# aurianer/DLA-Future

Measured on AMD Instinct MI355X. Metric: fp64 Cholesky TFlop/s, higher is better.
Workload: dtype f64

## Files before the change

### dla_future_amd/csrc/device/device_api.hpp

```cpp
#pragma once
#include <hip/hip_runtime.h>

#include "common.hpp"

namespace dlaf_mi355x {

inline hipError_t zero_device_now(void* p, size_t bytes) {
  hipError_t e = hipMemsetAsync(p, 0, bytes, nullptr);
  if (e == hipSuccess)
    e = hipStreamSynchronize(nullptr);
  return e;
}


constexpr int kDiagBlock = 64;
constexpr int kInfoSchedulingFailure = -1000000;

template <class T>
struct UpdateArgs {
  T* c;
  long c_tsr, c_tsc;
  int ldc;
  const T* a;
  long a_ts;
  int lda;
  const T* b;
  long b_ts;
  int ldb;
  int il0, il1, jl0, jl1;
  int nb, K;
  int pr, ri, pc, ci;
  int nt, last_rows;
  const int* info;
  int rect = 0;
  int nt_c = 0, last_cols = 0;
  int b_period = 1;
  long b_ts2 = 0;
  int b_jl0 = -1;
  int K1 = 0;
  const T* a2 = nullptr;
  const T* b2 = nullptr;
  int her2k = 0;
};
template <class T>
void launch_update(const UpdateArgs<T>& args, hipStream_t stream, int role = 0, long max_blocks = 0,
                   unsigned* counters = nullptr, bool counters_are_zero = false, long excl_slots = 0);
template <class T>
int update_blocks_per_cu();

template <class T>
struct TrsmArgs {
  T* b;
  long b_ts;
  int ldb;
  int il0, il1;
  int pr, ri;
  int nb, nt, last_rows;
  const T* l;
  int ldl;
  const T* winv;
  int n;
  const int* info;
  int upper = 0;
  int prio = 0;
};
template <class T>
void launch_trsm(const TrsmArgs<T>& args, hipStream_t stream);

template <class T>
void launch_potrf_diag(T* a, int lda, int jb, T* winv_block, int* info, int info_base, hipStream_t stream,
                       bool factor = true, bool upper = false, bool unit = false);

template <class T>
void launch_invert_diag_blocks(const T* tile, int ld, int kb, T* winv, int* info, hipStream_t stream, bool upper,
                               bool unit);

template <class T>
void launch_potrf_coop(T* tile, int ld, int kb, T* winv, int* info, int info_base, unsigned* sync,
                       hipStream_t stream, bool sync_is_zero = false, bool count_strips = true);
void update_launch_stats(long* persistent, long* exclusive);
unsigned long long* potrf_coop_trace_buffer();
inline size_t potrf_coop_sync_words(int kb) {
  const size_t g = (size_t) ((kb + kDiagBlock - 1) / kDiagBlock);
  return g + g * g;
}

template <class T>
struct LayoutArgs {
  T* tiles;
  T* cm;
  long ld_cm;
  int ltr, ltc;
  int nb;
  long rows, cols;
  int pr, ri, pc, ci;
  int transpose;
  int full = 0, conj = 0, scale = 0;
  T alpha{};
  int jl_first = 0, jl_count = 0;
  int rev_rows = 0, rev_cols = 0;
};
template <class T>
void launch_to_tiles(const LayoutArgs<T>& args, hipStream_t stream);
template <class T>
void launch_from_tiles(const LayoutArgs<T>& args, hipStream_t stream);

template <class T>
void launch_copy2d(T* dst, long ldd, const T* src, long lds, int rows, int cols, int transpose, int mask,
                   hipStream_t stream);

template <class T>
void launch_tile_xform(T* dst, long ldd, long dstride, const T* src, long lds, long sstride, int rows, int cols,
// ... 16 lines not shown
```

### dla_future_amd/csrc/device/kernels_potrf_coop.hip

```cpp
#include <cstdio>
#include <cstdlib>

#include "potrf_diag_core.hpp"

namespace dlaf_mi355x {

constexpr int kCB = kDiagBlock;

template <class T>
struct CoopCfg {
  using R = real_t<T>;
  static constexpr bool CX = TypeInfo<T>::is_complex;
  static constexpr int NPL = CX ? 2 : 1;
  static constexpr bool REGA = CX && sizeof(R) == 8;
  static constexpr int PAD = 16;
  static constexpr int LD = kCB + PAD;
  static constexpr int IMG = kCB * LD;
  static constexpr int OPERANDS = (REGA ? 1 : 2) * NPL * IMG;
  static constexpr int DIAG = diag_lds_elems<T, REGA>();
  static constexpr int ELEMS = OPERANDS > DIAG ? OPERANDS : DIAG;
  static constexpr int LDS_BYTES = ELEMS * (int) sizeof(R);
  static_assert(!REGA || LDS_BYTES <= 95 * 1024, "must fit beside one bulk-update workgroup");
};

// ... 538 lines not shown
        }
      }
      coop_poison_winv<T>(winv + (long) s * kCB * kCB);
      coop_publish(&flag[s], kCoopFailed, false);
      return;
    }
    T* Ws = winv + (long) s * kCB * kCB;
    for (int idx = t; idx < kPD * kPD; idx += kThreads) {
      const int rr = idx % kPD, cl = idx / kPD;
      if (rr < jb && cl < jb && rr >= cl) {
        R imv = 0;
        if constexpr (C::CX)
          imv = Lim[cl * kPDLd + rr];
        Ass[rr + (long) cl * ld] = make_el<T>(Lre[cl * kPDLd + rr], imv);
      }
      R wre = 0, wim = 0;
      if (rr < jb && cl < jb) {
        wre = diag_w_get<PACK>(Wre, PACK ? diag_wd_re<T, PACK>(Wre) : nullptr, rr, cl);
        if constexpr (C::CX)
          wim = diag_w_get<PACK>(Wim, PACK ? diag_wd_im<T, PACK>(Wre) : nullptr, rr, cl);
      }
      store_wt(&Ws[rr + (long) cl * kPD], make_el<T>(wre, wim));
    }
    coop_publish(&flag[s], 1u, false);
    if (trace != nullptr && s < 2 && t == 0)
      trace[16 + s * 8 + 6] = 4;
  }
}

template <class T>
__global__ __launch_bounds__(kThreads, 2) void potrf_coop_kernel(T* __restrict__ tile, int ld, int kb,
                                                                  T* __restrict__ winv, int* info, int info_base,
                                                                  unsigned* sync, long spin_limit, int prio, int* cu_busy,
                                                                  unsigned long long* trace) {
  int* mine = nullptr;
  if (cu_busy != nullptr && threadIdx.x == 0) {
    unsigned xcc;
    const unsigned key = phys_cu_key(xcc);
    mine = cu_busy + (xcc * 256u + key);
    atomicAdd(mine, 1);
  }
  potrf_coop_body<T>(tile, ld, kb, winv, info, info_base, sync, spin_limit, prio, trace);
  __syncthreads();
  if (mine != nullptr)
    atomicSub(mine, 1);
}

static int coop_wave_prio() {
  static const int p = [] {
    const char* e = std::getenv("DLAF_MI355X_POTRF_PRIO");
    return e ? std::atoi(e) : 1;
  }();
  return p;
}

int* cu_busy_table();

static unsigned long long* g_potrf_trace = nullptr;
unsigned long long* potrf_coop_trace_buffer() {
  static const bool on = [] {
    const char* e = std::getenv("DLAF_MI355X_POTRF_TRACE");
    return e && std::atoi(e) != 0;
  }();
  if (on && g_potrf_trace == nullptr) {
    if (hipMalloc(reinterpret_cast<void**>(&g_potrf_trace), 32 * sizeof(unsigned long long)) != hipSuccess ||
        zero_device_now(g_potrf_trace, 32 * sizeof(unsigned long long)) != hipSuccess) {
      (void) hipGetLastError();
      g_potrf_trace = nullptr;
    }
  }
  return g_potrf_trace;
}

static void fatal_device_config(const char* what) {
  std::fprintf(stderr, "[dlaf_mi355x] %s\n", what);
  std::abort();
}

template <class T>
void launch_potrf_coop(T* tile, int ld, int kb, T* winv, int* info, int info_base, unsigned* sync,
                       hipStream_t stream, bool sync_is_zero, bool count_strips) {
  if (kb <= 0)
    return;
  const int G = (kb + kCB - 1) / kCB;
  if (G > kThreads)
    fatal_device_config("potrf_coop: more than 256 strips per tile");
  if (!sync_is_zero)
    (void) hipMemsetAsync(sync, 0, sizeof(unsigned) * ((size_t) G + (size_t) G * G), stream);
  hipLaunchKernelGGL((potrf_coop_kernel<T>), dim3((unsigned) G), dim3(kThreads), CoopCfg<T>::LDS_BYTES, stream, tile, ld,
                     kb, winv, info, info_base, sync, coop_spin_limit(), coop_wave_prio(), count_strips ? cu_busy_table() : nullptr,
                     info_base == 0 ? potrf_coop_trace_buffer() : nullptr);
}

template <class T>
static void coop_init_one() {
  (void) hipFuncSetAttribute(reinterpret_cast<const void*>(&potrf_coop_kernel<T>),
                             hipFuncAttributeMaxDynamicSharedMemorySize, CoopCfg<T>::LDS_BYTES);
}

void potrf_coop_kernels_init() {
  coop_init_one<float>();
  coop_init_one<double>();
  coop_init_one<cfloat>();
  coop_init_one<cdouble>();
}

template void launch_potrf_coop<float>(float*, int, int, float*, int*, int, unsigned*, hipStream_t, bool, bool);
template void launch_potrf_coop<double>(double*, int, int, double*, int*, int, unsigned*, hipStream_t, bool, bool);
template void launch_potrf_coop<cfloat>(cfloat*, int, int, cfloat*, int*, int, unsigned*, hipStream_t, bool, bool);
template void launch_potrf_coop<cdouble>(cdouble*, int, int, cdouble*, int*, int, unsigned*, hipStream_t, bool, bool);

}
```

### dla_future_amd/csrc/device/kernels_update.hip

```cpp
#include <algorithm>
#include <cstdio>
#include <cstdlib>
#include <cstring>
#include <type_traits>
#include <utility>
#include <vector>

#include "device_api.hpp"
#include "mma_core.hpp"

namespace dlaf_mi355x {

template <class T>
struct UpdateCfg;
template <>
struct UpdateCfg<float> {
  using type = BlockCfg<float, 128, 128, 64, 64, 16>;
  static constexpr int min_waves = 2;
};
template <>
struct UpdateCfg<double> {
#if defined(DLAF_UPD_BIG)
  using type = BlockCfg<double, 256, 128, 64, 64, 16, true, DLAF_UPD_BIG, 512>;
  static constexpr int min_waves = 2;
// ... 10 lines not shown
};
template <>
struct UpdateCfg<cfloat> {
  using type = BlockCfg<cfloat, 128, 128, 64, 64, 16>;
  static constexpr int min_waves = 2;
};
template <>
struct UpdateCfg<cdouble> {
  using type = BlockCfg<cdouble, 128, 64, 64, 32, 8, true, 3>;
  static constexpr int min_waves = 2;
};

constexpr int kMaxPatchCols = 256;

struct UpdateMap {
  int ps;
  int psc;
  int PR;
  int tri;
  int PC;
  int colstart[kMaxPatchCols + 1];
  int xcd;
  int RB, CB;
  int bpt_m, bpt_n;
  long total;
  int persist;
  unsigned* counters;
  int lockstep;
  unsigned kphase_ticks;
  int excl_rank;
  unsigned excl_budget;
  int steal;
  int* cu_busy;
};

__device__ unsigned char g_cu_rank[8][256];

__global__ void cu_probe_kernel(unsigned* seen) {
  extern __shared__ unsigned char probe_lds[];
  if (threadIdx.x == 0) {
    unsigned xcc;
    const unsigned key = phys_cu_key(xcc);
    atomicOr(&seen[xcc * 8 + (key >> 5)], 1u << (key & 31));
    probe_lds[0] = (unsigned char) key;
  }
  for (int i = 0; i < 64; ++i)
    __builtin_amdgcn_s_sleep(64);
}

template <class T, bool VEC, bool UTAIL = false, int PART = 0>
__device__ __forceinline__ void update_block(const UpdateArgs<T>& p, const UpdateMap& mp, long w,
                                             real_t<T>* __restrict__ lds, int s0 = 0) {
  using Cfg = typename UpdateCfg<T>::type;
  using R = real_t<T>;

  const int ps = mp.ps, psc = mp.psc;
  const long patch = w >> (ps + psc);
  const int q = (int) (w & ((1 << (ps + psc)) - 1));
  int pi, pj;
  if (mp.tri) {
    int lo = 0, hi = mp.PC;
    while (hi - lo > 1) {
      const int mid = (lo + hi) >> 1;
      if (mp.colstart[mid] <= patch)
        lo = mid;
      else
        hi = mid;
// ... 249 lines not shown
            const T cv = col[ml];
            if constexpr (Cfg::CX) {
              T r{cv.re - acc.re[i][j][v], cv.im - acc.im[i][j][v]};
              if (diag && (m0 + ml) == (n0 + nl))
                r.im = R(0);
              col[ml] = r;
            }
            else {
              col[ml] = cv - acc.re[i][j][v];
            }
          }
        }
      }
    }
  }
}

template <class T, bool VEC, int ROLE>
__global__ __launch_bounds__(UpdateCfg<T>::type::THREADS, UpdateCfg<T>::min_waves) void update_kernel(UpdateArgs<T> p,
                                                                                                     UpdateMap mp) {
  using R = real_t<T>;
  extern __shared__ __attribute__((aligned(16))) unsigned char lds_raw[];
  R* lds = reinterpret_cast<R*>(lds_raw);
  if (*p.info != 0)
    return;
  if (!mp.persist) {
    const long v = blockIdx.x;
    const long w = mp.xcd ? (v & 7) * (mp.total >> 3) + (v >> 3) : v;
#ifdef DLAF_UPD_LEAN
    update_block<T, VEC, false, (ROLE == 0 ? 1 : 0)>(p, mp, w, lds);
#else
    update_block<T, VEC>(p, mp, w, lds);
#endif
    return;
  }
  __shared__ unsigned next_item;
  const int nq = mp.xcd ? 8 : 1;
  const long per_q = mp.total / nq;
  const int q0 = mp.xcd ? (int) (blockIdx.x & 7) : 0;
  const unsigned W = gridDim.x / nq;
  if (mp.excl_rank > 0) {
    __shared__ int leave;
    if (threadIdx.x == 0) {
      unsigned xcc;
      const unsigned key = phys_cu_key(xcc);
      leave = 0;
      if ((int) g_cu_rank[xcc][key] < mp.excl_rank)
        leave = atomicAdd(&mp.counters[15], 1u) < mp.excl_budget ? 1 : 0;
    }
    __syncthreads();
    if (leave)
      return;
  }
  __shared__ int next_s0;
  const int nslab = p.K / UpdateCfg<T>::type::BK;
  int q = q0, tried = 1;
  int* my_busy = nullptr;
  if (mp.cu_busy != nullptr && threadIdx.x == 0) {
    unsigned xcc;
    const unsigned key = phys_cu_key(xcc);
    my_busy = mp.cu_busy + (xcc * 256u + key);
  }
  for (;;) {
    if (threadIdx.x == 0) {
      if (my_busy != nullptr) {
        int spins = 0;
        while (__hip_atomic_load(my_busy, __ATOMIC_RELAXED, __HIP_MEMORY_SCOPE_AGENT) > 0 && ++spins < 4000)
          __builtin_amdgcn_s_sleep(64);
      }
      next_item = atomicAdd(&mp.counters[q], 1u);
      next_s0 = (mp.kphase_ticks != 0 && nslab > 1) ? (int) ((wall_clock64() / mp.kphase_ticks) % (unsigned) nslab) : 0;
    }
    __syncthreads();
#if DLAF_GLDS_SCALAR_ADDR
    const long i = (long) (unsigned) __builtin_amdgcn_readfirstlane((int) next_item);
    const int s0 = __builtin_amdgcn_readfirstlane(next_s0);
#else
    const long i = next_item;
    const int s0 = next_s0;
#endif
    __syncthreads();
    if (i >= per_q) {
      if (!mp.steal || tried >= nq)
        break;
      ++tried;
      q = (q + 1) % nq;
      continue;
    }
    if (mp.lockstep) {
      if (threadIdx.x == 0) {
        const unsigned need = (unsigned) (i / W) * W;
        long spins = 0;
        while (__hip_atomic_load(&mp.counters[8 + q], __ATOMIC_RELAXED, __HIP_MEMORY_SCOPE_AGENT) < need && ++spins < 2000000)
          __builtin_amdgcn_s_sleep(8);
      }
      __syncthreads();
    }
#ifdef DLAF_UPD_LEAN
    update_block<T, VEC, ROLE == 0, (ROLE == 0 ? 1 : 0)>(p, mp, (long) q * per_q + i, lds, s0);
#else
    update_block<T, VEC, ROLE == 0>(p, mp, (long) q * per_q + i, lds, s0);
#endif
    if (mp.lockstep && threadIdx.x == 0)
      __hip_atomic_fetch_add(&mp.counters[8 + q], 1u, __ATOMIC_RELAXED, __HIP_MEMORY_SCOPE_AGENT);
  }
}

static bool update_lockstep() {
  static const bool on = [] {
    const char* e = std::getenv("DLAF_MI355X_LOCKSTEP");
    return e ? std::atoi(e) != 0 : false;
  }();
  return on;
}

template <class T>
static unsigned kphase_ticks(int resident) {
  using Cfg = typename UpdateCfg<T>::type;
  static const double rate = [] {
    const char* on = std::getenv("DLAF_MI355X_KPHASE");
    if (on == nullptr || std::atoi(on) == 0)
      return 0.0;
    if (const char* e = std::getenv("DLAF_MI355X_KPHASE_RATE"))
      return std::atof(e) * 1e12;
    return (sizeof(real_t<T>) == 8 ? 66.5e12 : 120e12);
  }();
  static const double khz = [] {
    int dev = 0, v = 0;
    (void) hipGetDevice(&dev);
    if (hipDeviceGetAttribute(&v, hipDeviceAttributeWallClockRate, dev) != hipSuccess || v <= 0)
      v = 100000;
    return (double) v;
  }();
  if (rate <= 0 || resident <= 0)
    return 0;
// ... 11 lines not shown
static int* g_cu_busy = nullptr;
int* cu_busy_table() {
  static const bool on = [] {
    const char* e = std::getenv("DLAF_MI355X_POTRF_YIELD");
    return e ? std::atoi(e) != 0 : true;
  }();
  if (on && g_cu_busy == nullptr) {
    if (hipMalloc(reinterpret_cast<void**>(&g_cu_busy), 8 * 256 * sizeof(int)) != hipSuccess ||
        zero_device_now(g_cu_busy, 8 * 256 * sizeof(int)) != hipSuccess) {
      (void) hipGetLastError();
      g_cu_busy = nullptr;
    }
  }
  return g_cu_busy;
}

static int g_probe_xcds = 0, g_probe_cus_per_xcd = 0, g_probe_engines = 1;

static long g_launch_stats[2] = {0, 0};
void update_launch_stats(long* persistent, long* exclusive) {
  *persistent = g_launch_stats[0];
  *exclusive = g_launch_stats[1];
}

static bool update_steal() {
  static const bool on = [] {
    const char* e = std::getenv("DLAF_MI355X_STEAL");
    return e ? std::atoi(e) != 0 : true;
  }();
  return on;
}

template <class T>
void launch_update(const UpdateArgs<T>& a, hipStream_t stream, int role, long max_blocks, unsigned* counters,
                   bool counters_are_zero, long excl_slots) {
  using Cfg = typename UpdateCfg<T>::type;
  if (a.il1 <= a.il0 || a.jl1 <= a.jl0 || a.K <= 0 || a.nb <= 0)
    return;
  UpdateMap mp;
  mp.bpt_m = (a.nb + Cfg::BM - 1) / Cfg::BM;
  mp.bpt_n = (a.nb + Cfg::BN - 1) / Cfg::BN;
  mp.RB = (a.il1 - a.il0) * mp.bpt_m;
  mp.CB = (a.jl1 - a.jl0) * mp.bpt_n;
  static_assert(Cfg::BM % Cfg::BN == 0 && ((Cfg::BM / Cfg::BN) & (Cfg::BM / Cfg::BN - 1)) == 0, "BM = 2^s * BN");
  constexpr int kAspectShift = (Cfg::BM / Cfg::BN == 1) ? 0 : (Cfg::BM / Cfg::BN == 2) ? 1 : 2;
  const bool big = (mp.RB >= 16 && mp.CB >= 16);
  mp.ps = big ? 3 : 0;
  mp.psc = big ? 3 + kAspectShift : 0;
  mp.PR = (mp.RB + (1 << mp.ps) - 1) >> mp.ps;
  mp.PC = (mp.CB + (1 << mp.psc) - 1) >> mp.psc;
  long npatch = (long) mp.PR * mp.PC;
  mp.tri = 0;
  if (mp.PC <= kMaxPatchCols) {
    mp.tri = 1;
    mp.colstart[0] = 0;
    for (int pj = 0; pj < mp.PC; ++pj) {
      const int jl_min = a.jl0 + (pj << mp.psc) / mp.bpt_n;
      const long gj_min = (long) jl_min * a.pc + a.ci;
      long il_first = (gj_min - a.ri + a.pr - 1) / a.pr;
      if (gj_min <= a.ri || a.rect)
        il_first = 0;
      if (il_first < a.il0)
        il_first = a.il0;
      int cnt = 0;
      if (il_first < a.il1) {
        const int pi0 = (int) (((il_first - a.il0) * mp.bpt_m) >> mp.ps);
        cnt = mp.PR - pi0;
      }
      mp.colstart[pj + 1] = mp.colstart[pj] + cnt;
    }
    npatch = mp.colstart[mp.PC];
    if (npatch == 0)
      return;
  }
  mp.total = npatch << (mp.ps + mp.psc);
  mp.xcd = (mp.ps > 0) ? 1 : 0;
  long grid = mp.total;
  mp.persist = 0;
  mp.lockstep = 0;
  mp.kphase_ticks = 0;
  mp.counters = nullptr;
  mp.excl_rank = 0;
  mp.excl_budget = 0;
  mp.steal = 0;
  long excl_rank = 0;
  if (excl_slots > 0) {
    static const int per_cu = update_blocks_per_cu<T>();
    const long round = (long) per_cu * g_probe_xcds * g_probe_engines;
    if (g_probe_xcds > 0 && !update_lockstep() && excl_slots % round == 0 &&
        (excl_slots / round) * g_probe_engines <= g_probe_cus_per_xcd / 2)
      excl_rank = (excl_slots / round) * g_probe_engines;
    else {
      max_blocks = std::max<long>(8, max_blocks - excl_slots);
      excl_slots = 0;
    }
  }
  if (max_blocks > 0 && counters != nullptr && mp.total > max_blocks) {
    grid = mp.xcd ? (max_blocks / 8) * 8 : max_blocks;
    if (grid < 8)
      grid = 8;
    mp.persist = 1;
    mp.counters = counters;
    mp.lockstep = update_lockstep() ? 1 : 0;
    mp.kphase_ticks = kphase_ticks<T>((int) (grid));
    mp.steal = (update_steal() && !mp.lockstep) ? 1 : 0;
    mp.cu_busy = (role == 0) ? g_cu_busy : nullptr;
    ++g_launch_stats[0];
    if (excl_rank > 0) {
      mp.excl_rank = (int) excl_rank;
      mp.excl_budget = (unsigned) excl_slots;
      ++g_launch_stats[1];
    }
    if (!counters_are_zero)
      (void) hipMemsetAsync(counters, 0, 16 * sizeof(unsigned), stream);
  }
  const bool vec = aligned16<T>(a.a, a.lda) && aligned16<T>(a.a, a.a_ts) && aligned16<T>(a.b, a.ldb) &&
                   aligned16<T>(a.b, a.b_ts) && aligned16<T>(a.b, a.b_ts2) &&
                   (a.K1 == 0 || (aligned16<T>(a.a2, 0) && aligned16<T>(a.b2, 0)));
  auto go = [&](auto vtag, auto rtag) {
    constexpr bool V = decltype(vtag)::value;
    constexpr int RL = decltype(rtag)::value;
    hipLaunchKernelGGL((update_kernel<T, V, RL>), dim3((unsigned) grid), dim3(Cfg::THREADS), Cfg::LDS_BYTES, stream, a, mp);
  };
  auto by_role = [&](auto vtag) {
    switch (role) {
      case 0: go(vtag, std::integral_constant<int, 0>{}); break;
      case 1: go(vtag, std::integral_constant<int, 1>{}); break;
      case 3: go(vtag, std::integral_constant<int, 3>{}); break;
      default: go(vtag, std::integral_constant<int, 2>{}); break;
    }
  };
  if (vec)
    by_role(std::true_type{});
  else
    by_role(std::false_type{});
}

template <class T>
int update_blocks_per_cu() {
  using Cfg = typename UpdateCfg<T>::type;
  int n = 0;
  if (hipOccupancyMaxActiveBlocksPerMultiprocessor(&n, reinterpret_cast<const void*>(&update_kernel<T, true, 0>), Cfg::THREADS,
                                                   Cfg::LDS_BYTES) != hipSuccess || n < 1)
    n = 1;
  return n;
}

template <class T>
static void update_init_one() {
  using Cfg = typename UpdateCfg<T>::type;
#define SET_ONE(V, RL)                                                                         \
  (void) hipFuncSetAttribute(reinterpret_cast<const void*>(&update_kernel<T, V, RL>),           \
                             hipFuncAttributeMaxDynamicSharedMemorySize, Cfg::LDS_BYTES)
  SET_ONE(true, 0);
  SET_ONE(true, 1);
  SET_ONE(true, 2);
  SET_ONE(true, 3);
  SET_ONE(false, 0);
  SET_ONE(false, 1);
  SET_ONE(false, 2);
  SET_ONE(false, 3);
#undef SET_ONE
}

static void probe_compute_units() {
  const bool verbose = [] {
    const char* e = std::getenv("DLAF_MI355X_PROBE_VERBOSE");
    return e && std::atoi(e) != 0;
// ... 56 lines not shown
    max_engines = std::max(max_engines, engines);
    {
      std::vector<unsigned> sorted(keys.size());
      for (size_t r = 0; r < idx.size(); ++r)
        sorted[r] = keys[idx[r]];
      keys.swap(sorted);
    }
    if (verbose) {
      std::fprintf(stderr, "[dlaf_mi355x] compute-unit probe: XCD %d: %zu compute units:", x, keys.size());
      for (unsigned k : keys)
        std::fprintf(stderr, " %u.%u.%u", k >> 5, (k >> 4) & 1u, k & 15u);
      std::fprintf(stderr, "\n");
    }
  }
  if (xcds == 0)
    return note("no compute unit seen", hipSuccess);
  err = hipMemcpyToSymbol(HIP_SYMBOL(g_cu_rank), rank, sizeof(rank));
  if (err != hipSuccess)
    return note("hipMemcpyToSymbol", err);
  g_probe_xcds = xcds;
  g_probe_cus_per_xcd = min_cus;
  g_probe_engines = std::max(1, max_engines);
}

void update_kernels_init() {
  update_init_one<float>();
  update_init_one<double>();
  update_init_one<cfloat>();
  update_init_one<cdouble>();
  probe_compute_units();
  (void) cu_busy_table();
}

template void launch_update<float>(const UpdateArgs<float>&, hipStream_t, int, long, unsigned*, bool, long);
template int update_blocks_per_cu<float>();
template void launch_update<double>(const UpdateArgs<double>&, hipStream_t, int, long, unsigned*, bool, long);
template int update_blocks_per_cu<double>();
template void launch_update<cfloat>(const UpdateArgs<cfloat>&, hipStream_t, int, long, unsigned*, bool, long);
template int update_blocks_per_cu<cfloat>();
template void launch_update<cdouble>(const UpdateArgs<cdouble>&, hipStream_t, int, long, unsigned*, bool, long);
template int update_blocks_per_cu<cdouble>();

}
```

### dla_future_amd/csrc/host/cholesky.cpp

```cpp
#include "runtime.hpp"

#include <algorithm>
#include <cstdlib>
#include <cstring>
#include <vector>

namespace dlaf_mi355x {

static bool potrf_use_chain() {
  static const bool chain = [] {
    const char* e = std::getenv("DLAF_MI355X_POTRF");
    return e && std::strcmp(e, "chain") == 0;
  }();
  return chain;
}

template <class T>
void potrf_tile(T* t, int ld, int kb, T* winv, int* info, int info_base, unsigned* sync, hipStream_t s) {
  constexpr int JB = kDiagBlock;
  if (!potrf_use_chain()) {
    launch_potrf_coop(t, ld, kb, winv, info, info_base, sync, s,  true,  true);
    return;
  }
  for (int j0 = 0; j0 < kb; j0 += JB) {
    const int jb = std::min(JB, kb - j0);
    T* djj = t + j0 + (size_t) j0 * ld;
    T* wj = winv + (size_t) (j0 / JB) * JB * JB;
    launch_potrf_diag(djj, ld, jb, wj, info, info_base + j0, s);
    const int rem = kb - j0 - jb;
    if (rem <= 0)
      break;
    T* sub = t + (j0 + jb) + (size_t) j0 * ld;
    TrsmArgs<T> ta;
    ta.b = sub;
    ta.b_ts = 0;
    ta.ldb = ld;
    ta.il0 = 0;
    ta.il1 = 1;
    ta.pr = 1;
    ta.ri = 0;
    ta.nb = rem;
    ta.nt = 1;
    ta.last_rows = rem;
    ta.l = djj;
    ta.ldl = ld;
    ta.winv = wj;
    ta.n = jb;
    ta.info = info;
    launch_trsm(ta, s);
    UpdateArgs<T> ua;
    ua.c = t + (j0 + jb) + (size_t) (j0 + jb) * ld;
    ua.c_tsr = ua.c_tsc = 0;
    ua.ldc = ld;
    ua.a = sub;
    ua.a_ts = 0;
    ua.lda = ld;
// ... 153 lines not shown
  }

  StepT one_panel(long k, long il_n, long jl_n, const T* a_base) const {
    return StepT::one_panel(m.rows.tile_extent(k), il_n, jl_n, a_base, m.tile_elems);
  }

  void update_work(long il0, long il1, long j0, long j1, int kb, double& flops, double& bytes) const {
    flops = bytes = 0;
    const double cx = TypeInfo<T>::is_complex ? 4.0 : 1.0;
    for (long jl = j0; jl < j1; ++jl) {
      const long gj = m.cols.global_of(jl);
      const double nj = m.rows.tile_extent(gj);
      for (long il = std::max(il0, m.rows.next_local(gj)); il < il1; ++il) {
        const long gi = m.rows.global_of(il);
        const double mi = m.rows.tile_extent(gi);
        if (gi == gj) {
          flops += cx * mi * (mi + 1) * kb;
          bytes += (mi * kb + mi * mi) * sizeof(T);
        }
        else {
          flops += cx * 2.0 * mi * nj * kb;
          bytes += (mi * kb + nj * kb + 2.0 * mi * nj) * sizeof(T);
        }
      }
    }
  }

  double column_flops(const StepT& st, long jl) const {
    double f, by;
    update_work(std::max(st.il_n, m.rows.next_local(m.cols.global_of(jl))), m.ltr, jl, jl + 1, st.kb, f, by);
    return f;
  }

  void update(const StepT& st, long j0, long j1, hipStream_t s, int role, long reserve, long il_from = -1,
              long il_to = -1, int kind = -1) {
    if (!st.valid || j0 >= j1)
      return;
    const long il0 = std::max(std::max(st.il_n, il_from), m.rows.next_local(m.cols.global_of(j0)));
    const long il1 = il_to < 0 ? m.ltr : std::min(il_to, m.ltr);
    if (il0 >= il1)
      return;
    UpdateArgs<T> ua;
    ua.c = m.tiles;
    ua.c_tsr = (long) m.tile_elems;
    ua.c_tsc = (long) (m.tile_elems * m.ltr);
    ua.ldc = m.nb;
    ua.a = st.a_base + (size_t) (il0 - st.il_n) * m.tile_elems;
    ua.a_ts = (long) m.tile_elems;
    ua.lda = m.nb;
    ua.b = st.b_base;
    ua.b_ts = st.b_ts;
    ua.b_period = st.b_period;
    ua.b_ts2 = st.b_ts2;
    ua.b_jl0 = (int) st.jl_n;
    if (st.k1 > 0) {
      ua.K1 = st.k1;
      ua.a2 = st.a2_base + (size_t) (il0 - st.il_n) * m.tile_elems;
      ua.b2 = st.b2_base;
    }
    ua.ldb = m.nb;
    ua.il0 = (int) il0;
    ua.il1 = (int) il1;
    ua.jl0 = (int) j0;
    ua.jl1 = (int) j1;
    ua.nb = m.nb;
    ua.K = st.kb;
    ua.pr = m.rows.P;
    ua.ri = m.rows.shift();
    ua.pc = m.cols.P;
    ua.ci = m.cols.shift();
    ua.nt = (int) m.nt;
    ua.last_rows = last_rows;
    ua.info = m.info;
    double fl, by;
    update_work(il0, il1, j0, j1, st.kb, fl, by);
    const int pk = kind < 0 ? role : kind;
    m.prof_begin(pk, s);
    unsigned* cnt = m.coop_sync;
    bool zero = false;
    if (reserve > 0) {
      const size_t sl = std::min(next_update_slice, m.coop_sync_update_slices - 1);
      cnt = m.coop_sync + 16 * sl;
      zero = next_update_slice < m.coop_sync_update_slices - 1;
      ++next_update_slice;
    }
    static const bool exclusive = [] {
      const char* e = std::getenv("DLAF_MI355X_EXCLUSIVE_CUS");
      return e ? std::atoi(e) != 0 : true;
    }();
    if (reserve > 0 && exclusive)
      launch_update(ua, s, role, m.bulk_slots, cnt, zero, reserve);
    else
      launch_update(ua, s, role, reserve > 0 ? std::max<long>(8, m.bulk_slots - reserve) : 0, cnt, zero);
    DLAF_HIP_CHECK(hipGetLastError());
    m.prof_end(pk, s, fl, by);
  }

  void trsm(long il0, long il1, long klc, const T* Lkk, const T* Wkk, int kb, hipStream_t ts = nullptr) {
    if (ts == nullptr)
      ts = s_main;
    if (il0 >= il1)
      return;
    TrsmArgs<T> ta;
    ta.b = m.tile(il0, klc);
    ta.b_ts = (long) m.tile_elems;
    ta.ldb = m.nb;
    ta.il0 = (int) il0;
    ta.il1 = (int) il1;
    ta.pr = m.rows.P;
    ta.ri = m.rows.shift();
    ta.nb = m.nb;
    ta.nt = (int) m.nt;
    ta.last_rows = last_rows;
    ta.l = Lkk;
    ta.ldl = m.nb;
    ta.winv = Wkk;
    ta.n = kb;
    ta.info = m.info;
    ta.prio = (ts != s_main) ? 1 : 0;
    double fl = 0, by = 0;
    for (long il = il0; il < il1; ++il) {
      const double mi = m.rows.tile_extent(m.rows.global_of(il));
      fl += (TypeInfo<T>::is_complex ? 4.0 : 1.0) * (double) kb * kb * mi;
      by += (0.5 * kb * kb + 2.0 * mi * kb) * sizeof(T);
    }
    m.prof_begin(2, ts);
    launch_trsm(ta, ts);
    DLAF_HIP_CHECK(hipGetLastError());
    m.prof_end(2, ts, fl, by);
  }

  T* winv_of(long k) const { return m.winv + (size_t) (k & 1) * m.winv_elems(); }
  T* diag_ws_of(long k) const { return m.diag_ws + (size_t) (k & 1) * (m.tile_elems + m.winv_elems()); }
  void potrf(long k) {
    if (m.rows.rank != m.rows.owner(k) || m.cols.rank != m.cols.owner(k))
      return;
    const int kb = m.rows.tile_extent(k);
    const double cxf = TypeInfo<T>::is_complex ? 4.0 : 1.0;
    m.prof_begin(3, s_panel);
    potrf_tile(m.tile(m.rows.local_of(k), m.cols.local_of(k)), m.nb, kb, winv_of(k), m.info, (int) (k * m.nb),
               m.coop_sync + 16 * m.coop_sync_update_slices + m.coop_sync_potrf_words * (size_t) k, s_panel);
    DLAF_HIP_CHECK(hipGetLastError());
    m.prof_end(3, s_panel, cxf * (double) kb * kb * kb / 3.0, (double) kb * kb * sizeof(T));
  }

  void diag_bcast(long k, bool in_row, bool in_col, const T*& Lkk, const T*& Wkk) {
    Lkk = Wkk = nullptr;
    if (in_row && in_col) {
      Lkk = m.tile(m.rows.local_of(k), m.cols.local_of(k));
      Wkk = winv_of(k);
    }
    if (in_col && m.rows.P > 1) {
      T* ws = diag_ws_of(k);
      if (in_row) {
        DLAF_HIP_CHECK(hipMemcpyAsync(ws, Lkk, tile_bytes, hipMemcpyDeviceToDevice, s_panel));
        DLAF_HIP_CHECK(hipMemcpyAsync(ws + m.tile_elems, Wkk, m.winv_elems() * sizeof(T), hipMemcpyDeviceToDevice, s_panel));
      }
      DLAF_HIP_CHECK(hipEventRecord(m.ev_diag[k], s_panel));
      DLAF_HIP_CHECK(hipStreamWaitEvent(s_comm, m.ev_diag[k], 0));
      tr->bcast(ax_col, m.rows.owner(k), m.rows.rank, ws, ws, tile_bytes + m.winv_elems() * sizeof(T), s_comm);
      DLAF_HIP_CHECK(hipEventRecord(m.ev_diag[k], s_comm));
      Lkk = ws;
      Wkk = ws + m.tile_elems;
    }
    else {
      DLAF_HIP_CHECK(hipEventRecord(m.ev_diag[k], s_panel));
    }
  }

  void transposed_panel(StepT& cur, int buf) {
    if (m.rows.P > 1) {
      m.bcast_transposed_panel(tr, ax_col, cur.a_base, cur.il_n, cur.jl_n, m.panelT[buf], s_comm, cur.b_period,
                               cur.b_ts2);
      cur.b_base = m.panelT[buf];
// ... 36 lines not shown
        continue;
      const double t = t_of(cand);
      if (t < best_t) {
        best_t = t;
        best = cand;
      }
    }
    return best;
  }

  bool u1_on_main(long k, long slots, double bulk_flops) const {
    using R = PairRates<T>;
    const long nb = m.nb;
    const double cxf = TypeInfo<T>::is_complex ? 4.0 : 1.0;
    const double below1 = (double) std::max<long>(0, m.n - (k + 1) * nb), below2 = (double) std::max<long>(0, m.n - (k + 2) * nb);
    const double fl_chain = cxf * (double) nb * nb * (below1 + below2) + cxf * 2.0 * (double) nb * nb * below1;
    const double nblk = (double) nb / kDiagBlock;
    const double t_chain = 2.0 * nblk * nblk * R::t_potrf_blk2 + fl_chain / (R::r_trsm_slot * (double) slots);
    const double t_bulk = bulk_flops / (R::r_bulk * (1.0 - (double) slots / (double) m.bulk_slots));
    return t_bulk < t_chain;
  }

  void issue_pairs();
  void issue_sidecar();
  void issue_early();
  void issue_classic();
};

template <class T>
void CholeskyIssue<T>::issue_pairs() {
  constexpr double kSplitFrac = 0.3;
  const long nt = m.nt, ltr = m.ltr, ltc = m.ltc;
  StepT prev;
  for (long k = 0; k < nt; k += 2) {
    if (tr)
      tr->mark(k);
    if (k >= 2)
      DLAF_HIP_CHECK(hipStreamWaitEvent(s_panel, m.ev_high[k - 2], 0));
    potrf(k);
    const bool second = k + 1 < nt;
    const bool more = k + 2 < nt;
    if (second) {
      trsm(k + 1, ltr, k, m.tile(k, k), winv_of(k), m.rows.tile_extent(k), s_panel);
      panel_done(k, s_panel);
    }
    const bool bulk = prev.valid && prev.rest0 < ltc;
    std::vector<double> colfl;
    double bulk_flops = 0;
    for (long jl = bulk ? prev.rest0 : ltc; jl < ltc; ++jl) {
      colfl.push_back(column_flops(prev, jl));
      bulk_flops += colfl.back();
    }
    const long slots = bulk ? pair_slots(k, bulk_flops) : kSidecarSlots;
    const bool u1_main = second && (!bulk || u1_on_main(k, slots, bulk_flops));
    long splitA = prev.rest0;
    if (u1_main && bulk) {
      double acc = 0;
      while (splitA < ltc && acc < kSplitFrac * bulk_flops)
        acc += colfl[(size_t) (splitA++ - prev.rest0)];
    }
    update(prev, prev.rest0, splitA, s_main, 0, slots);
    if (second) {
      const StepT u1 = one_panel(k, k + 1, k + 1, m.tile(k + 1 < ltr ? k + 1 : 0, k));
      if (u1_main) {
        DLAF_HIP_CHECK(hipStreamWaitEvent(s_main, m.ev_panel[k], 0));
        update(u1, k + 1, k + 2, s_main, 1, 0);
        DLAF_HIP_CHECK(hipEventRecord(m.ev_head[k], s_main));
        DLAF_HIP_CHECK(hipStreamWaitEvent(s_panel, m.ev_head[k], 0));
      }
      else {
        update(u1, k + 1, k + 2, s_panel, 1, 0);
      }
      potrf(k + 1);
      if (more) {
        trsm(k + 2, ltr, k + 1, m.tile(k + 1, k + 1), winv_of(k + 1), m.rows.tile_extent(k + 1), s_panel);
        panel_done(k + 1, s_panel);
      }
    }
    update(prev, splitA, ltc, s_main, 0, slots);
    if (!more) {
      join_last_diag(k);
      break;
    }
    DLAF_HIP_CHECK(hipStreamWaitEvent(s_main, m.ev_panel[k + 1], 0));
    StepT cur = StepT::two_panels(m.rows.tile_extent(k), m.rows.tile_extent(k + 1), k + 2, m.tile(k + 2, k),
                                  m.tile(k + 2, k + 1), m.tile_elems);
    update(cur, k + 2, std::min<long>(k + 4, ltc), s_main, 1, 0);
    DLAF_HIP_CHECK(hipEventRecord(m.ev_high[k], s_main));
    cur.rest0 = std::min<long>(k + 4, ltc);
    prev = cur;
  }
}

template <class T>
void CholeskyIssue<T>::issue_sidecar() {
  const long nt = m.nt, ltr = m.ltr, ltc = m.ltc;
  StepT prev;
  for (long k = 0; k < nt; ++k) {
    const int kb = m.rows.tile_extent(k);
    if (tr)
      tr->mark(k);
    const long il_n = m.rows.next_local(k + 1), jl_n = m.cols.next_local(k + 1);
    const long klc = m.cols.local_of(k);
    if (k >= 1)
      DLAF_HIP_CHECK(hipStreamWaitEvent(s_panel, m.ev_high[k - 1], 0));
    potrf(k);
    if (k == nt - 1) {
      update(prev, prev.rest0, ltc, s_main, 0, kSidecarSlots);
      join_last_diag(k);
      break;
    }
    trsm(il_n, ltr, klc, m.tile(m.rows.local_of(k), klc), winv_of(k), kb, s_panel);
    panel_done(k, s_panel);
    update(prev, prev.rest0, ltc, s_main, 0, kSidecarSlots);
    DLAF_HIP_CHECK(hipStreamWaitEvent(s_main, m.ev_panel[k], 0));
    StepT cur = one_panel(k, il_n, jl_n, m.tile(il_n < ltr ? il_n : 0, klc));
    transposed_panel(cur, 0);
    cur.rest0 = jl_n;
    if (jl_n < ltc) {
      update(cur, jl_n, jl_n + 1, s_main, 1, 0);
      cur.rest0 = jl_n + 1;
    }
    DLAF_HIP_CHECK(hipEventRecord(m.ev_high[k], s_main));
// ... 137 lines not shown
void DeviceMatrix<T>::factorize_async() {
  CholeskyIssue<T> f(*this);
  const Schedule schedule = choose_schedule(f.dist, nb, TypeInfo<T>::is_complex);

  for (auto& ps : prof) {
    ps.used = 0;
    ps.flops = ps.bytes = ps.ms = 0;
    ps.launches = 0;
  }
  DLAF_HIP_CHECK(hipMemsetAsync(info, 0, sizeof(int), f.s_panel));
  DLAF_HIP_CHECK(hipMemsetAsync(coop_sync, 0, sizeof(unsigned) * coop_sync_words, f.s_panel));
  if (unsigned long long* tb = potrf_coop_trace_buffer())
    DLAF_HIP_CHECK(hipMemsetAsync(tb, 0, 32 * sizeof(unsigned long long), f.s_panel));
  DLAF_HIP_CHECK(hipEventRecord(ev_start[0], f.s_panel));
  DLAF_HIP_CHECK(hipStreamWaitEvent(f.s_main, ev_start[0], 0));
  DLAF_HIP_CHECK(hipStreamWaitEvent(f.s_comm, ev_start[0], 0));

  switch (schedule) {
    case Schedule::Pairs: f.issue_pairs(); break;
    case Schedule::Sidecar: f.issue_sidecar(); break;
    case Schedule::Early: f.issue_early(); break;
    case Schedule::Classic: f.issue_classic(); break;
  }

  DLAF_HIP_CHECK(hipEventRecord(ev_done[0], f.s_main));
  DLAF_HIP_CHECK(hipStreamWaitEvent(f.s_panel, ev_done[0], 0));
  DLAF_HIP_CHECK(hipMemcpyAsync(info_host, info, sizeof(int), hipMemcpyDeviceToHost, f.s_panel));
}

#define INST(T)                                                                                     \
  template void DeviceMatrix<T>::factorize_async();                                                 \
  template int DeviceMatrix<T>::bcast_transposed_panel(Transport*, CommAxis, const T*, long, long, T*, \
                                                       hipStream_t, int&, long&);                   \
  template void potrf_tile<T>(T*, int, int, T*, int*, int, unsigned*, hipStream_t);
INST(float)
INST(double)
INST(cfloat)
INST(cdouble)
#undef INST

}
```

### dla_future_amd/csrc/host/runtime.hpp

```cpp
#pragma once
#include <hip/hip_runtime.h>

#include <atomic>
#include <cstddef>
#include <cstdint>
#include <memory>
#include <vector>

#include "../device/device_api.hpp"
#include "distribution.hpp"

namespace dlaf_mi355x {

[[noreturn]] void fatal(const char* fmt, ...);

#define DLAF_HIP_CHECK(expr)                                                                     \
  do {                                                                                           \
    hipError_t e_ = (expr);                                                                      \
    if (e_ != hipSuccess)                                                                        \
      ::dlaf_mi355x::fatal("[dlaf_mi355x] HIP error %s at %s:%d: %s\n", hipGetErrorName(e_), __FILE__, \
                           __LINE__, #expr);                                                     \
  } while (0)

hipError_t pool_malloc(void** p, size_t bytes);
// ... 99 lines not shown
    long launches = 0;
  };
  ProfSlot prof[4];
  long bulk_slots = 0;
  bool profiling = true;
  void prof_begin(int kind, hipStream_t s);
  void prof_end(int kind, hipStream_t s, double flops, double bytes);

  int bcast_transposed_panel(Transport* tr, CommAxis ax_col, const T* a_base, long il_n, long jl_n, T* dst,
                             hipStream_t s, int& period, long& ts2);

  T* tile(long il, long jl) const { return tiles + (size_t) (il + jl * ltr) * tile_elems; }
  size_t winv_elems() const { return (size_t) ((nb + kDiagBlock - 1) / kDiagBlock) * kDiagBlock * kDiagBlock; }

  void create(Grid* g, char uplo_, long n_, int nb_, int isrc, int jsrc);
  void destroy();
  ~DeviceMatrix() override { destroy(); }

  void upload(const T* host, long ld);
  void download(T* host, long ld, bool staging_is_current = false);
  void copy_from(const DeviceMatrix<T>& other);
  void residual_of(DeviceMatrix<T>& factor, double* max_diff, double* max_a);
  int factorize();
  int factorize_and_download(T* host, long ld);
  std::atomic<long> panels_issued{-1};
  void factorize_async();
  int wait();
  int local_info = 0;
  bool fetch_tile(long gi, long gj, T* host, long ld);
  double trsm_profile(int reps, double* flops, double* bytes);
};

template <class T>
void potrf_tile(T* t, int ld, int kb, T* winv, int* info, int info_base, unsigned* sync, hipStream_t s);

template <class T>
int tile_potrf(char uplo, int n, T* a, int lda);
template <class T>
void tile_trsm(char uplo, int m, int n, const T* a, int lda, T* b, int ldb);
template <class T>
void tile_herk(char uplo, int n, int k, const T* a, int lda, T* c, int ldc);
template <class T>
void tile_gemm(char uplo, int m, int n, int k, const T* a, int lda, const T* b, int ldb, T* c, int ldc);

int grid_selftest(Grid& g, size_t bytes);

template <class T>
int triangular_solver_host(Grid* g, char side, char uplo, char op, char diag, T alpha, const T* a, long lda, int a_isrc,
                           int a_jsrc, T* b, long ldb, long m, long n, int nb, int b_isrc, int b_jsrc, int nb_free = 0);

void solver_last_profile(double* ms, double* flops);

MatrixBase* general_matrix_create(Grid* g, char type, long m, long n, int nb, int isrc, int jsrc);
void general_matrix_transfer(MatrixBase* h, void* host, long ld, bool upload);
int triangular_solver_device(char side, char uplo, char op, char diag, const void* alpha, MatrixBase* a, MatrixBase* b);

template <class T>
int gen_to_std_device(DeviceMatrix<T>& a, DeviceMatrix<T>& l);
template <class T>
int gen_to_std_host(Grid* g, char uplo, T* a, long lda, const T* l, long ldl, long n, int nb, int isrc, int jsrc);

void runtime_init();
void runtime_finalize();
bool runtime_initialized();

}
```

Baseline: 68.96.

## Fuse lookahead update into bulk update and gate diagonal potrf on device counter

The separate high-priority lookahead update launch and its event wait are replaced in the sidecar path. The bulk update kernel now schedules the head columns (the lookahead tiles) first and bumps a device counter after each head item finishes. The cooperative potrf kernel is launched immediately and spins on that counter until the head items are complete. This removes a kernel launch and a stream event dependency from the critical path, so the diagonal factorization can start as soon as its inputs are ready. The cost is busy-wait spinning by potrf workgroups that occupy CUs, and a risk of scheduling deadlock, which is handled by a spin limit that raises an error code.

Result: no change. 69.32 (median of 6 runs) (+0.5%).

```diff
diff --git a/dla_future_amd/csrc/device/device_api.hpp b/dla_future_amd/csrc/device/device_api.hpp
--- a/dla_future_amd/csrc/device/device_api.hpp
+++ b/dla_future_amd/csrc/device/device_api.hpp
@@ -43,8 +43,9 @@
   int her2k = 0;
 };
 template <class T>
-void launch_update(const UpdateArgs<T>& args, hipStream_t stream, int role = 0, long max_blocks = 0,
-                   unsigned* counters = nullptr, bool counters_are_zero = false, long excl_slots = 0);
+long launch_update(const UpdateArgs<T>& args, hipStream_t stream, int role = 0, long max_blocks = 0,
+                   unsigned* counters = nullptr, bool counters_are_zero = false, long excl_slots = 0,
+                   int head_cols = 0, unsigned* head_done = nullptr);
 template <class T>
 int update_blocks_per_cu();
 
@@ -77,7 +78,8 @@
 
 template <class T>
 void launch_potrf_coop(T* tile, int ld, int kb, T* winv, int* info, int info_base, unsigned* sync,
-                       hipStream_t stream, bool sync_is_zero = false, bool count_strips = true);
+                       hipStream_t stream, bool sync_is_zero = false, bool count_strips = true,
+                       const unsigned* wait_word = nullptr, unsigned wait_target = 0);
 void update_launch_stats(long* persistent, long* exclusive);
 unsigned long long* potrf_coop_trace_buffer();
 inline size_t potrf_coop_sync_words(int kb) {
diff --git a/dla_future_amd/csrc/device/kernels_potrf_coop.hip b/dla_future_amd/csrc/device/kernels_potrf_coop.hip
--- a/dla_future_amd/csrc/device/kernels_potrf_coop.hip
+++ b/dla_future_amd/csrc/device/kernels_potrf_coop.hip
@@ -594,7 +594,25 @@
 __global__ __launch_bounds__(kThreads, 2) void potrf_coop_kernel(T* __restrict__ tile, int ld, int kb,
                                                                   T* __restrict__ winv, int* info, int info_base,
                                                                   unsigned* sync, long spin_limit, int prio, int* cu_busy,
-                                                                  unsigned long long* trace) {
+                                                                  unsigned long long* trace, const unsigned* wait_word,
+                                                                  unsigned wait_target) {
+  if (wait_word != nullptr) {
+    if (threadIdx.x == 0) {
+      long spins = 0;
+      while (__hip_atomic_load(wait_word, __ATOMIC_RELAXED, __HIP_MEMORY_SCOPE_AGENT) < wait_target) {
+        if (__hip_atomic_load(info, __ATOMIC_RELAXED, __HIP_MEMORY_SCOPE_AGENT) != 0)
+          break;
+        __builtin_amdgcn_s_sleep(32);
+        if (++spins > spin_limit) {
+          atomicCAS(info, 0, kInfoSchedulingFailure);
+          break;
+        }
+      }
+      __builtin_amdgcn_fence(__ATOMIC_ACQUIRE, "agent");
+      asm volatile("s_waitcnt vmcnt(0)" ::: "memory");
+    }
+    __syncthreads();
+  }
   int* mine = nullptr;
   if (cu_busy != nullptr && threadIdx.x == 0) {
     unsigned xcc;
@@ -641,7 +659,8 @@
 
 template <class T>
 void launch_potrf_coop(T* tile, int ld, int kb, T* winv, int* info, int info_base, unsigned* sync,
-                       hipStream_t stream, bool sync_is_zero, bool count_strips) {
+                       hipStream_t stream, bool sync_is_zero, bool count_strips, const unsigned* wait_word,
+                       unsigned wait_target) {
   if (kb <= 0)
     return;
   const int G = (kb + kCB - 1) / kCB;
@@ -651,7 +670,8 @@
     (void) hipMemsetAsync(sync, 0, sizeof(unsigned) * ((size_t) G + (size_t) G * G), stream);
   hipLaunchKernelGGL((potrf_coop_kernel<T>), dim3((unsigned) G), dim3(kThreads), CoopCfg<T>::LDS_BYTES, stream, tile, ld,
                      kb, winv, info, info_base, sync, coop_spin_limit(), coop_wave_prio(), count_strips ? cu_busy_table() : nullptr,
-                     info_base == 0 ? potrf_coop_trace_buffer() : nullptr);
+                     info_base == 0 ? potrf_coop_trace_buffer() : nullptr, wait_target > 0 ? wait_word : nullptr,
+                     wait_target);
 }
 
 template <class T>
@@ -667,9 +687,9 @@
   coop_init_one<cdouble>();
 }
 
-template void launch_potrf_coop<float>(float*, int, int, float*, int*, int, unsigned*, hipStream_t, bool, bool);
-template void launch_potrf_coop<double>(double*, int, int, double*, int*, int, unsigned*, hipStream_t, bool, bool);
-template void launch_potrf_coop<cfloat>(cfloat*, int, int, cfloat*, int*, int, unsigned*, hipStream_t, bool, bool);
-template void launch_potrf_coop<cdouble>(cdouble*, int, int, cdouble*, int*, int, unsigned*, hipStream_t, bool, bool);
-
-}
+template void launch_potrf_coop<float>(float*, int, int, float*, int*, int, unsigned*, hipStream_t, bool, bool, const unsigned*, unsigned);
+template void launch_potrf_coop<double>(double*, int, int, double*, int*, int, unsigned*, hipStream_t, bool, bool, const unsigned*, unsigned);
+template void launch_potrf_coop<cfloat>(cfloat*, int, int, cfloat*, int*, int, unsigned*, hipStream_t, bool, bool, const unsigned*, unsigned);
+template void launch_potrf_coop<cdouble>(cdouble*, int, int, cdouble*, int*, int, unsigned*, hipStream_t, bool, bool, const unsigned*, unsigned);
+
+}
diff --git a/dla_future_amd/csrc/device/kernels_update.hip b/dla_future_amd/csrc/device/kernels_update.hip
--- a/dla_future_amd/csrc/device/kernels_update.hip
+++ b/dla_future_amd/csrc/device/kernels_update.hip
@@ -66,7 +66,18 @@
   unsigned excl_budget;
   int steal;
   int* cu_busy;
+  long head;
+  unsigned* head_done;
 };
+
+__device__ __forceinline__ void publish_head_item(unsigned* head_done) {
+  asm volatile("s_waitcnt vmcnt(0)" ::: "memory");
+  __syncthreads();
+  if (threadIdx.x == 0) {
+    __builtin_amdgcn_fence(__ATOMIC_RELEASE, "agent");
+    __hip_atomic_fetch_add(head_done, 1u, __ATOMIC_RELAXED, __HIP_MEMORY_SCOPE_AGENT);
+  }
+}
 
 __device__ unsigned char g_cu_rank[8][256];
 
@@ -382,11 +393,14 @@
 #else
     update_block<T, VEC>(p, mp, w, lds);
 #endif
+    if (w < mp.head)
+      publish_head_item(mp.head_done);
     return;
   }
   __shared__ unsigned next_item;
   const int nq = mp.xcd ? 8 : 1;
   const long per_q = mp.total / nq;
+  const long head_q = mp.head / nq;
   const int q0 = mp.xcd ? (int) (blockIdx.x & 7) : 0;
   const unsigned W = gridDim.x / nq;
   if (mp.excl_rank > 0) {
@@ -446,11 +460,14 @@
       }
       __syncthreads();
     }
+    const long w = i < head_q ? q * head_q + i : mp.head + q * (per_q - head_q) + (i - head_q);
 #ifdef DLAF_UPD_LEAN
-    update_block<T, VEC, ROLE == 0, (ROLE == 0 ? 1 : 0)>(p, mp, (long) q * per_q + i, lds, s0);
+    update_block<T, VEC, ROLE == 0, (ROLE == 0 ? 1 : 0)>(p, mp, w, lds, s0);
 #else
-    update_block<T, VEC, ROLE == 0>(p, mp, (long) q * per_q + i, lds, s0);
-#endif
+    update_block<T, VEC, ROLE == 0>(p, mp, w, lds, s0);
+#endif
+    if (i < head_q)
+      publish_head_item(mp.head_done);
     if (mp.lockstep && threadIdx.x == 0)
       __hip_atomic_fetch_add(&mp.counters[8 + q], 1u, __ATOMIC_RELAXED, __HIP_MEMORY_SCOPE_AGENT);
   }
@@ -528,11 +545,11 @@
 }
 
 template <class T>
-void launch_update(const UpdateArgs<T>& a, hipStream_t stream, int role, long max_blocks, unsigned* counters,
-                   bool counters_are_zero, long excl_slots) {
+long launch_update(const UpdateArgs<T>& a, hipStream_t stream, int role, long max_blocks, unsigned* counters,
+                   bool counters_are_zero, long excl_slots, int head_cols, unsigned* head_done) {
   using Cfg = typename UpdateCfg<T>::type;
   if (a.il1 <= a.il0 || a.jl1 <= a.jl0 || a.K <= 0 || a.nb <= 0)
-    return;
+    return 0;
   UpdateMap mp;
   mp.bpt_m = (a.nb + Cfg::BM - 1) / Cfg::BM;
   mp.bpt_n = (a.nb + Cfg::BN - 1) / Cfg::BN;
@@ -567,9 +584,18 @@
     }
     npatch = mp.colstart[mp.PC];
     if (npatch == 0)
-      return;
+      return 0;
   }
   mp.total = npatch << (mp.ps + mp.psc);
+  mp.head = 0;
+  mp.head_done = head_done;
+  if (head_cols > 0 && head_done != nullptr) {
+    mp.head = mp.total;
+    if (mp.tri) {
+      const int pc_end = std::min(mp.PC, (int) (((long) head_cols * mp.bpt_n + (1 << mp.psc) - 1) >> mp.psc));
+      mp.head = (long) mp.colstart[pc_end] << (mp.ps + mp.psc);
+    }
+  }
   mp.xcd = (mp.ps > 0) ? 1 : 0;
   long grid = mp.total;
   mp.persist = 0;
@@ -630,6 +656,7 @@
     by_role(std::true_type{});
   else
     by_role(std::false_type{});
+  return mp.head;
 }
 
 template <class T>
@@ -752,13 +779,13 @@
   (void) cu_busy_table();
 }
 
-template void launch_update<float>(const UpdateArgs<float>&, hipStream_t, int, long, unsigned*, bool, long);
+template long launch_update<float>(const UpdateArgs<float>&, hipStream_t, int, long, unsigned*, bool, long, int, unsigned*);
 template int update_blocks_per_cu<float>();
-template void launch_update<double>(const UpdateArgs<double>&, hipStream_t, int, long, unsigned*, bool, long);
+template long launch_update<double>(const UpdateArgs<double>&, hipStream_t, int, long, unsigned*, bool, long, int, unsigned*);
 template int update_blocks_per_cu<double>();
-template void launch_update<cfloat>(const UpdateArgs<cfloat>&, hipStream_t, int, long, unsigned*, bool, long);
+template long launch_update<cfloat>(const UpdateArgs<cfloat>&, hipStream_t, int, long, unsigned*, bool, long, int, unsigned*);
 template int update_blocks_per_cu<cfloat>();
-template void launch_update<cdouble>(const UpdateArgs<cdouble>&, hipStream_t, int, long, unsigned*, bool, long);
+template long launch_update<cdouble>(const UpdateArgs<cdouble>&, hipStream_t, int, long, unsigned*, bool, long, int, unsigned*);
 template int update_blocks_per_cu<cdouble>();
 
 }
diff --git a/dla_future_amd/csrc/host/cholesky.cpp b/dla_future_amd/csrc/host/cholesky.cpp
--- a/dla_future_amd/csrc/host/cholesky.cpp
+++ b/dla_future_amd/csrc/host/cholesky.cpp
@@ -16,12 +16,16 @@
 }
 
 template <class T>
-void potrf_tile(T* t, int ld, int kb, T* winv, int* info, int info_base, unsigned* sync, hipStream_t s) {
+void potrf_tile(T* t, int ld, int kb, T* winv, int* info, int info_base, unsigned* sync, hipStream_t s,
+                const unsigned* wait_word, unsigned wait_target) {
   constexpr int JB = kDiagBlock;
   if (!potrf_use_chain()) {
-    launch_potrf_coop(t, ld, kb, winv, info, info_base, sync, s,  true,  true);
+    launch_potrf_coop(t, ld, kb, winv, info, info_base, sync, s,  true,  true,
+                      wait_word, wait_target);
     return;
   }
+  if (wait_target > 0)
+    fatal("[dlaf_mi355x] potrf_tile: the multi-launch form cannot wait on a device counter\n");
   for (int j0 = 0; j0 < kb; j0 += JB) {
     const int jb = std::min(JB, kb - j0);
     T* djj = t + j0 + (size_t) j0 * ld;
@@ -241,14 +245,20 @@
     return f;
   }
 
-  void update(const StepT& st, long j0, long j1, hipStream_t s, int role, long reserve, long il_from = -1,
-              long il_to = -1, int kind = -1) {
+  unsigned* take_slice() {
+    if (next_update_slice >= m.coop_sync_update_slices - 1)
+      fatal("[dlaf_mi355x] factorization: out of pre-zeroed counter slices\n");
+    return m.coop_sync + 16 * next_update_slice++;
+  }
+
+  long update(const StepT& st, long j0, long j1, hipStream_t s, int role, long reserve, long il_from = -1,
+              long il_to = -1, int kind = -1, int head_cols = 0, unsigned* head_done = nullptr) {
     if (!st.valid || j0 >= j1)
-      return;
+      return 0;
     const long il0 = std::max(std::max(st.il_n, il_from), m.rows.next_local(m.cols.global_of(j0)));
     const long il1 = il_to < 0 ? m.ltr : std::min(il_to, m.ltr);
     if (il0 >= il1)
-      return;
+      return 0;
     UpdateArgs<T> ua;
     ua.c = m.tiles;
     ua.c_tsr = (long) m.tile_elems;
@@ -297,12 +307,15 @@
       const char* e = std::getenv("DLAF_MI355X_EXCLUSIVE_CUS");
       return e ? std::atoi(e) != 0 : true;
     }();
+    long head = 0;
     if (reserve > 0 && exclusive)
-      launch_update(ua, s, role, m.bulk_slots, cnt, zero, reserve);
+      head = launch_update(ua, s, role, m.bulk_slots, cnt, zero, reserve, head_cols, head_done);
     else
-      launch_update(ua, s, role, reserve > 0 ? std::max<long>(8, m.bulk_slots - reserve) : 0, cnt, zero);
+      head = launch_update(ua, s, role, reserve > 0 ? std::max<long>(8, m.bulk_slots - reserve) : 0, cnt, zero, 0,
+                           head_cols, head_done);
     DLAF_HIP_CHECK(hipGetLastError());
     m.prof_end(pk, s, fl, by);
+    return head;
   }
 
   void trsm(long il0, long il1, long klc, const T* Lkk, const T* Wkk, int kb, hipStream_t ts = nullptr) {
@@ -341,14 +354,15 @@
 
   T* winv_of(long k) const { return m.winv + (size_t) (k & 1) * m.winv_elems(); }
   T* diag_ws_of(long k) const { return m.diag_ws + (size_t) (k & 1) * (m.tile_elems + m.winv_elems()); }
-  void potrf(long k) {
+  void potrf(long k, const unsigned* wait_word = nullptr, long wait_target = 0) {
     if (m.rows.rank != m.rows.owner(k) || m.cols.rank != m.cols.owner(k))
       return;
     const int kb = m.rows.tile_extent(k);
     const double cxf = TypeInfo<T>::is_complex ? 4.0 : 1.0;
     m.prof_begin(3, s_panel);
     potrf_tile(m.tile(m.rows.local_of(k), m.cols.local_of(k)), m.nb, kb, winv_of(k), m.info, (int) (k * m.nb),
-               m.coop_sync + 16 * m.coop_sync_update_slices + m.coop_sync_potrf_words * (size_t) k, s_panel);
+               m.coop_sync + 16 * m.coop_sync_update_slices + m.coop_sync_potrf_words * (size_t) k, s_panel,
+               wait_word, (unsigned) wait_target);
     DLAF_HIP_CHECK(hipGetLastError());
     m.prof_end(3, s_panel, cxf * (double) kb * kb * kb / 3.0, (double) kb * kb * sizeof(T));
   }
@@ -451,18 +465,12 @@
   constexpr double kSplitFrac = 0.3;
   const long nt = m.nt, ltr = m.ltr, ltc = m.ltc;
   StepT prev;
+  long la1 = 0;
   for (long k = 0; k < nt; k += 2) {
     if (tr)
       tr->mark(k);
-    if (k >= 2)
-      DLAF_HIP_CHECK(hipStreamWaitEvent(s_panel, m.ev_high[k - 2], 0));
-    potrf(k);
     const bool second = k + 1 < nt;
     const bool more = k + 2 < nt;
-    if (second) {
-      trsm(k + 1, ltr, k, m.tile(k, k), winv_of(k), m.rows.tile_extent(k), s_panel);
-      panel_done(k, s_panel);
-    }
     const bool bulk = prev.valid && prev.rest0 < ltc;
     std::vector<double> colfl;
     double bulk_flops = 0;
@@ -478,7 +486,26 @@
       while (splitA < ltc && acc < kSplitFrac * bulk_flops)
         acc += colfl[(size_t) (splitA++ - prev.rest0)];
     }
-    update(prev, prev.rest0, splitA, s_main, 0, slots);
+    const long first_end = u1_main ? splitA : ltc;
+    unsigned* head_done = nullptr;
+    long head = 0;
+    if (prev.valid) {
+      if (!potrf_use_chain() && slots == kSidecarSlots) {
+        head_done = take_slice();
+        head = update(prev, prev.jl_n, first_end, s_main, 0, slots, -1, -1, -1, (int) (la1 - prev.jl_n), head_done);
+      }
+      else {
+        update(prev, prev.jl_n, la1, s_main, 1, 0);
+        DLAF_HIP_CHECK(hipEventRecord(m.ev_high[k - 2], s_main));
+        DLAF_HIP_CHECK(hipStreamWaitEvent(s_panel, m.ev_high[k - 2], 0));
+        update(prev, prev.rest0, first_end, s_main, 0, slots);
+      }
+    }
+    potrf(k, head_done, head);
+    if (second) {
+      trsm(k + 1, ltr, k, m.tile(k, k), winv_of(k), m.rows.tile_extent(k), s_panel);
+      panel_done(k, s_panel);
+    }
     if (second) {
       const StepT u1 = one_panel(k, k + 1, k + 1, m.tile(k + 1 < ltr ? k + 1 : 0, k));
       if (u1_main) {
@@ -496,18 +523,16 @@
         panel_done(k + 1, s_panel);
       }
     }
-    update(prev, splitA, ltc, s_main, 0, slots);
+    update(prev, std::max(first_end, prev.rest0), ltc, s_main, 0, slots);
     if (!more) {
       join_last_diag(k);
       break;
     }
     DLAF_HIP_CHECK(hipStreamWaitEvent(s_main, m.ev_panel[k + 1], 0));
-    StepT cur = StepT::two_panels(m.rows.tile_extent(k), m.rows.tile_extent(k + 1), k + 2, m.tile(k + 2, k),
-                                  m.tile(k + 2, k + 1), m.tile_elems);
-    update(cur, k + 2, std::min<long>(k + 4, ltc), s_main, 1, 0);
-    DLAF_HIP_CHECK(hipEventRecord(m.ev_high[k], s_main));
-    cur.rest0 = std::min<long>(k + 4, ltc);
-    prev = cur;
+    prev = StepT::two_panels(m.rows.tile_extent(k), m.rows.tile_extent(k + 1), k + 2, m.tile(k + 2, k),
+                             m.tile(k + 2, k + 1), m.tile_elems);
+    la1 = std::min<long>(k + 4, ltc);
+    prev.rest0 = la1;
   }
 }
 
@@ -711,7 +736,7 @@
   template void DeviceMatrix<T>::factorize_async();                                                 \
   template int DeviceMatrix<T>::bcast_transposed_panel(Transport*, CommAxis, const T*, long, long, T*, \
                                                        hipStream_t, int&, long&);                   \
-  template void potrf_tile<T>(T*, int, int, T*, int*, int, unsigned*, hipStream_t);
+  template void potrf_tile<T>(T*, int, int, T*, int*, int, unsigned*, hipStream_t, const unsigned*, unsigned);
 INST(float)
 INST(double)
 INST(cfloat)
diff --git a/dla_future_amd/csrc/host/runtime.hpp b/dla_future_amd/csrc/host/runtime.hpp
--- a/dla_future_amd/csrc/host/runtime.hpp
+++ b/dla_future_amd/csrc/host/runtime.hpp
@@ -155,7 +155,8 @@
 };
 
 template <class T>
-void potrf_tile(T* t, int ld, int kb, T* winv, int* info, int info_base, unsigned* sync, hipStream_t s);
+void potrf_tile(T* t, int ld, int kb, T* winv, int* info, int info_base, unsigned* sync, hipStream_t s,
+                const unsigned* wait_word = nullptr, unsigned wait_target = 0);
 
 template <class T>
 int tile_potrf(char uplo, int n, T* a, int lda);
```
